# swook/EVE

Measured on AMD Instinct MI355X. Metric: train-step frames/sec, 128x128 eye patches T=30, higher is better.
Workload: dtype bf16; 1 GPU; BASELINE configs[1]: EyeNet training (configs/eye_net.json: ResNet-18-IN + GRU-128, angular + pupil L1 losses, clip 5.0, Adam wd 0.005), 128x128 patches, fwd+bwd+clip+Adam; global_batch=32, batch_per_gpu=32, seq_len=30, parallelism=dp1

## Files before the change

eve_amd/csrc/conv_igemm.hip:

```cpp
#include <limits.h>
#include <stdio.h>
#include <stdlib.h>

#include <initializer_list>
#include <type_traits>
#include "common.h"

namespace eve {

struct GatherParams {
    int N, IH, IW, Cin;
    int OH, OW, Cout;
    int KH, KW;
    int o_mul, k_mul, off, div;
    int K;
    uint32_t M;
    FastDiv fd_ohw, fd_ow, fd_cin, fd_kw, fd_oh;
};

template <typename T>
__device__ __forceinline__ uint4 prologue_vec(uint4 q, const float* __restrict__ ssp, int act) {
    constexpr int VEC = Elem<T>::VEC;
    float f[VEC];
    Elem<T>::unpack(q, f);
    const float4* s4 = reinterpret_cast<const float4*>(ssp);
#pragma unroll
    for (int e = 0; e < VEC / 2; ++e) {
        float4 s = s4[e];
        f[2 * e] = act_fwd(f[2 * e] * s.x + s.y, act);
        f[2 * e + 1] = act_fwd(f[2 * e + 1] * s.z + s.w, act);
    }
    return Elem<T>::pack(f);
}

template <typename T> struct Mma {
    __device__ static __forceinline__ void run(f32x4_t& acc, const uint4& a, const uint4& b) { Elem<T>::mfma(acc, a, b); }
};
template <> struct Mma<float> {
    __device__ static __forceinline__ void run(f32x4_t& acc, const uint4& a, const uint4& b) {
        acc = __builtin_amdgcn_mfma_f32_16x16x4f32(__builtin_bit_cast(float, a.x), __builtin_bit_cast(float, b.x), acc, 0, 0, 0);
        acc = __builtin_amdgcn_mfma_f32_16x16x4f32(__builtin_bit_cast(float, a.y), __builtin_bit_cast(float, b.y), acc, 0, 0, 0);
        acc = __builtin_amdgcn_mfma_f32_16x16x4f32(__builtin_bit_cast(float, a.z), __builtin_bit_cast(float, b.z), acc, 0, 0, 0);
        acc = __builtin_amdgcn_mfma_f32_16x16x4f32(__builtin_bit_cast(float, a.w), __builtin_bit_cast(float, b.w), acc, 0, 0, 0);
    }
};

}
#include "conv_fast.h"
#include "conv_wg8.h"
#include "conv_wg8s2.h"
#include "conv_ws64.h"
#include "conv_1x1.h"
#include "conv_3x3s.h"
#include "wgrad_halo.h"
#include "wgrad_wg8.h"
namespace eve {

template <typename T, int NT, bool PRO>
__global__ __launch_bounds__(256) void igemm_kernel(const GatherParams p, const T* __restrict__ src,
                                                    const T* __restrict__ w,
                                                    const float* __restrict__ bias,
                                                    const float* __restrict__ ss, const int pro_act,
                                                    const int epi_act, T* __restrict__ out) {
    constexpr int VEC = Elem<T>::VEC;
    constexpr int BM = 128, BN = 32 * NT, BK = 8 * VEC;
    __shared__ uint4 lds[2 * (BM + BN) * 8];

    const int tid = threadIdx.x;
    const uint32_t tiles_n = (p.Cout + BN - 1) / BN;
    const uint32_t lid = xcd_remap(blockIdx.x, gridDim.x);
    const uint32_t m0 = (lid / tiles_n) * BM;
    const uint32_t n0 = (lid % tiles_n) * BN;

    const int v = tid & 7;
    const int r0 = tid >> 3;
    int a_y0[4], a_x0[4], a_pix[4], a_n[4];
    bool a_ok[4];
#pragma unroll
    for (int j = 0; j < 4; ++j) {
        const uint32_t m = m0 + r0 + 32 * j;
        a_ok[j] = m < p.M;
        const uint32_t mm = a_ok[j] ? m : 0;
        const uint32_t n = fd_div(mm, p.fd_ohw);
        const uint32_t rem = mm - n * (uint32_t)(p.OH * p.OW);
        const uint32_t oy = fd_div(rem, p.fd_ow);
        const uint32_t ox = rem - oy * (uint32_t)p.OW;
        a_y0[j] = (int)oy * p.o_mul + p.off;
        a_x0[j] = (int)ox * p.o_mul + p.off;
        a_pix[j] = (int)n * p.IH * p.IW;
        a_n[j] = (int)n;
    }

    uint4 ra[4], rb[NT];

    auto load_tile = [&](int kt) {
        const uint32_t kvec = (uint32_t)kt * BK + (uint32_t)v * VEC;
        const bool kvalid = kvec < (uint32_t)p.K;
        const uint32_t tap = fd_div(kvec, p.fd_cin);
        const int ci = (int)(kvec - tap * (uint32_t)p.Cin);
        const uint32_t kh = fd_div(tap, p.fd_kw);
        const int kw = (int)(tap - kh * (uint32_t)p.KW);
        const int dy = (int)kh * p.k_mul, dx = kw * p.k_mul;
#pragma unroll
        for (int j = 0; j < 4; ++j) {
            int sy = a_y0[j] + dy, sx = a_x0[j] + dx;
            bool ok = a_ok[j] && kvalid && sy >= 0 && sx >= 0;
            if (p.div > 1) {
                ok = ok && (sy % p.div == 0) && (sx % p.div == 0);
                sy /= p.div;
                sx /= p.div;
            }
            ok = ok && sy < p.IH && sx < p.IW;
            uint4 q = make_uint4(0, 0, 0, 0);
            if (ok) {
                const size_t e = ((size_t)(a_pix[j] + sy * p.IW + sx)) * (size_t)p.Cin + (size_t)ci;
                q = *reinterpret_cast<const uint4*>(src + e);
                if (PRO) q = prologue_vec<T>(q, ss + ((size_t)a_n[j] * p.Cin + ci) * 2, pro_act);
            }
            ra[j] = q;
        }
#pragma unroll
        for (int j = 0; j < NT; ++j) {
            const uint32_t co = n0 + r0 + 32 * j;
            uint4 q = make_uint4(0, 0, 0, 0);
            if (kvalid && co < (uint32_t)p.Cout)
                q = *reinterpret_cast<const uint4*>(w + (size_t)co * p.K + kvec);
            rb[j] = q;
        }
    };
    auto store_tile = [&](int buf) {
        uint4* base = lds + buf * (BM + BN) * 8;
#pragma unroll
        for (int j = 0; j < 4; ++j) {
            const int row = r0 + 32 * j;
            base[row * 8 + (v ^ (row & 7))] = ra[j];
        }
#pragma unroll
        for (int j = 0; j < NT; ++j) {
            const int row = r0 + 32 * j;
            base[BM * 8 + row * 8 + (v ^ (row & 7))] = rb[j];
        }
    };

    const int lane = tid & 63, wv = tid >> 6;
    const int wm = wv >> 1, wn = wv & 1;
    const int li = lane & 15, lg = lane >> 4;

    f32x4_t acc[4][NT];
#pragma unroll
    for (int a = 0; a < 4; ++a)
#pragma unroll
        for (int b = 0; b < NT; ++b) acc[a][b] = f32x4_t{0.f, 0.f, 0.f, 0.f};

    constexpr bool SPLIT_SUM = std::is_same<T, float>::value;
    constexpr int FLUSH = 8;
    f32x4_t tot[SPLIT_SUM ? 4 : 1][SPLIT_SUM ? NT : 1];
    if (SPLIT_SUM) {
#pragma unroll
        for (int a = 0; a < 4; ++a)
#pragma unroll
            for (int b = 0; b < NT; ++b) tot[SPLIT_SUM ? a : 0][SPLIT_SUM ? b : 0] = f32x4_t{0.f, 0.f, 0.f, 0.f};
    }

    const int nk = (p.K + BK - 1) / BK;
    load_tile(0);
    store_tile(0);
    __syncthreads();
    for (int kt = 0; kt < nk; ++kt) {
        const int cur = kt & 1;
        const bool more = kt + 1 < nk;
        if (more) load_tile(kt + 1);
        if (SPLIT_SUM && kt > 0 && (kt % FLUSH) == 0) {
#pragma unroll
            for (int a = 0; a < 4; ++a)
#pragma unroll
                for (int b = 0; b < NT; ++b) {
                    tot[SPLIT_SUM ? a : 0][SPLIT_SUM ? b : 0] += acc[a][b];
                    acc[a][b] = f32x4_t{0.f, 0.f, 0.f, 0.f};
                }
        }
        const uint4* la = lds + cur * (BM + BN) * 8;
        const uint4* lb = la + BM * 8;
#pragma unroll
        for (int c = 0; c < 2; ++c) {
            const int vc = c * 4 + lg;
            uint4 fx[4], fw[NT];
#pragma unroll
            for (int mt = 0; mt < 4; ++mt) {
                const int row = wm * 64 + mt * 16 + li;
                fx[mt] = la[row * 8 + (vc ^ (row & 7))];
            }
#pragma unroll
            for (int nt = 0; nt < NT; ++nt) {
                const int row = wn * 16 * NT + nt * 16 + li;
                fw[nt] = lb[row * 8 + (vc ^ (row & 7))];
            }
#pragma unroll
            for (int mt = 0; mt < 4; ++mt)
#pragma unroll
                for (int nt = 0; nt < NT; ++nt) Mma<T>::run(acc[mt][nt], fw[nt], fx[mt]);
        }
        if (more) store_tile(cur ^ 1);
        __syncthreads();
    }

    if (SPLIT_SUM) {
#pragma unroll
        for (int a = 0; a < 4; ++a)
// ... 410 lines not shown
        tp.ntaps = p.KH * p.KW;
        for (int kh = 0; kh < p.KH; ++kh)
            for (int kw = 0; kw < p.KW; ++kw) {
                const int t = kh * p.KW + kw;
                tp.dy[t] = (signed char)(kh * p.k_mul); tp.dx[t] = (signed char)(kw * p.k_mul); tp.wt[t] = (signed char)t;
            }
        tp.osy = tp.osx = 1; tp.oy0 = tp.ox0 = 0; tp.OHf = p.OH; tp.OWf = p.OW;
        launch_dma_one<T>(p, tp, src, w, bias, epi_act, out, (uint32_t)src_bytes, (uint32_t)w_bytes, s);
        return true;
    }
    if (p.o_mul != 1 || p.k_mul != -1 || bias || (epi_act & 0xff) != EVE_ACT_NONE) return false;
    const int sd = p.div;
    bool need_zero = false;
    for (int pass = 0; pass < 2; ++pass) {
        for (int py = 0; py < sd; ++py)
            for (int px = 0; px < sd; ++px) {
                TapPlan tp;
                tp.ntaps = 0;
                for (int kh = 0; kh < p.KH; ++kh)
                    for (int kw = 0; kw < p.KW; ++kw) {
                        const int ny = py + p.off - kh, nx = px + p.off - kw;
                        if (ny % sd != 0 || nx % sd != 0) continue;
                        tp.dy[tp.ntaps] = (signed char)(ny / sd); tp.dx[tp.ntaps] = (signed char)(nx / sd);
                        tp.wt[tp.ntaps] = (signed char)(kh * p.KW + kw);
                        ++tp.ntaps;
                    }
                const int sub_h = (p.OH - py + sd - 1) / sd, sub_w = (p.OW - px + sd - 1) / sd;
                if (sub_h <= 0 || sub_w <= 0) continue;
                if (tp.ntaps == 0) { need_zero = true; continue; }
                if (pass == 0) continue;
                GatherParams q = p;
                q.OH = sub_h; q.OW = sub_w;
                q.o_mul = 1; q.off = 0; q.div = 1;
                q.M = (uint32_t)((long long)p.N * sub_h * sub_w);
                q.fd_ohw = make_fastdiv(sub_h * sub_w); q.fd_ow = make_fastdiv(sub_w);
                tp.osy = tp.osx = sd; tp.oy0 = py; tp.ox0 = px; tp.OHf = p.OH; tp.OWf = p.OW;
                launch_dma_one<T>(q, tp, src, w, bias, epi_act, out, (uint32_t)src_bytes, (uint32_t)w_bytes, s);
            }
        if (pass == 0 && need_zero && !(epi_act & EVE_EPI_ACC))
            (void)hipMemsetAsync(out, 0, (size_t)p.N * p.OH * p.OW * p.Cout * sizeof(T), s);
    }
    return true;
}

template <typename T>
static int launch_igemm(const GatherParams& p, const void* src, const void* w, const float* bias,
                        const float* ss, int pro_act, int epi_act, void* out, hipStream_t s) {
    if (!ss && !use_v1() && launch_igemm_dma<T>(p, src, w, bias, epi_act, out, s)) return 0;
    const bool wide = p.Cout > 64;
    const uint32_t bn = wide ? 128 : 64;
    const uint32_t tiles = ((p.M + 127) / 128) * ((p.Cout + bn - 1) / bn);
    dim3 grid(tiles), block(256);
    const T* a = (const T*)src; const T* b = (const T*)w; T* o = (T*)out;
    if (wide) {
        if (ss) EVE_LAUNCH("igemm_kernel<T, 4, true>", (igemm_kernel<T, 4, true>), grid, block, 0, s, p, a, b, bias, ss, pro_act, epi_act, o);
        else    EVE_LAUNCH("igemm_kernel<T, 4, false>", (igemm_kernel<T, 4, false>), grid, block, 0, s, p, a, b, bias, ss, pro_act, epi_act, o);
    } else {
        if (ss) EVE_LAUNCH("igemm_kernel<T, 2, true>", (igemm_kernel<T, 2, true>), grid, block, 0, s, p, a, b, bias, ss, pro_act, epi_act, o);
        else    EVE_LAUNCH("igemm_kernel<T, 2, false>", (igemm_kernel<T, 2, false>), grid, block, 0, s, p, a, b, bias, ss, pro_act, epi_act, o);
    }
    return 0;
}

static void wgrad_split(const GatherParams& p, uint32_t tk, uint32_t tc, size_t lds_per_wg, uint32_t& splits, uint32_t& rows) {
    const int target_env = g_cfg.wgrad_target_wgs;
    uint32_t per_cu = lds_per_wg ? (uint32_t)((160 * 1024) / lds_per_wg) : 3;
    per_cu = per_cu < 1 ? 1 : (per_cu > 3 ? 3 : per_cu);
    const uint32_t target = target_env > 0 ? (uint32_t)target_env : 256u * per_cu;
    uint32_t want = target / (tk * tc);
    const int min_rows = g_cfg.wgrad_min_rows;
    uint32_t max_splits = (p.M + (uint32_t)min_rows - 1) / (uint32_t)min_rows;
    splits = want < 1 ? 1 : (want > max_splits ? max_splits : want);
    if (splits < 1) splits = 1;
    if (splits > 65535) splits = 65535;
    rows = (p.M + splits - 1) / splits;
    rows = (rows + 63) / 64 * 64;
    splits = (p.M + rows - 1) / rows;
}

template <typename HT>
static bool launch_wgrad_halo(const GatherParams& p, const void* x, const void* dy, float* dw, float* db, hipStream_t s) {
    if (!g_cfg.wgrad_halo) return false;
    const int ks = p.KH;
    if ((ks != 3 && ks != 1) || p.KW != ks || p.o_mul != 1 || p.k_mul != 1 || p.off != -(ks / 2) || p.div != 1 || p.OH != p.IH ||
        p.OW != p.IW)
        return false;
    const int W = p.IW, H = p.IH;
    const long long min_m = g_cfg.wgrad_halo_min_m;
    if (W < 32 || W > 128 || (W & (W - 1)) || p.Cin % 16 || p.Cout % 16 || (long long)p.M < min_m) return false;
    const int MT = p.Cout / 16, CT = p.Cin / 16;
    const bool split = ks == 3 && MT == 4 && CT == 4;
    if (ks == 3 && !split && !((MT == 1 && (CT == 1 || CT == 2 || CT == 4)) || (MT == 2 && (CT == 1 || CT == 2)))) return false;
    if (ks == 1 && !((MT == 2 && CT == 1) || (MT == 1 && CT == 4) || (MT == 1 && CT == 2) || (MT == 4 && CT == 2) || (MT == 2 && CT == 4)))
        return false;
    const unsigned long long xb = (unsigned long long)p.N * H * W * p.Cin * 2, db_ = (unsigned long long)p.M * p.Cout * 2;
    if (xb >= (1ull << 31) || db_ >= (1ull << 31)) return false;
    const size_t red = (size_t)(ks * ks * p.Cin * p.Cout + p.Cout) * 4;
    const unsigned occ = (ks == 3 && MT * CT >= 4) ? 2 : 3;
    int TH = 0; size_t lds = 0;
    int nreg = 0;
    if (split) {
        const int force_th = g_cfg.wg64_th, force_nreg = g_cfg.wg64_nreg;
        for (int th : {8, 4, 2, 1}) {
            if (force_th && th != force_th) continue;
            const size_t need = (size_t)(th + 2) * (W + 2) * 128 + (size_t)th * W * 128;
            for (int nr : {3, 2}) {
                if (force_nreg && nr != force_nreg) continue;
                if (nr * need <= (size_t)160 * 1024) { TH = th; nreg = nr; lds = nr * need > red ? nr * need : red; break; }
            }
            if (TH) break;
        }
    } else
    for (size_t budget : {(size_t)(occ == 3 ? 52 : 78) * 1024, (size_t)78 * 1024}) {
        for (int th : {4, 2, 1}) {
            const size_t need = (size_t)(th + ks - 1) * (W + ks - 1) * p.Cin * 2 + (size_t)th * W * p.Cout * 2;
            if (need <= budget && need >= red) { TH = th; lds = need; break; }
        }
        if (TH) break;
    }
    if (!TH) return false;
    WgradHaloParams h;
    h.N = p.N; h.H = H; h.W = W; h.TH = TH; h.bands = (H + TH - 1) / TH;
    h.total_bands = (uint32_t)p.N * h.bands; h.x_bytes = (uint32_t)xb; h.dy_bytes = (uint32_t)db_;
    h.log2_cpr = 0; h.nreg = nreg;
    while ((32 << h.log2_cpr) < W) ++h.log2_cpr;
    const unsigned per_cu = (unsigned)((160 * 1024) / lds);
    unsigned grid = 256 * (per_cu > occ ? occ : per_cu);
    if (grid > h.total_bands) grid = h.total_bands;
    auto band_tile = [&](auto kernel) { launch(kernel, dim3(grid), dim3(256), lds, s, h, (const HT*)x, (const HT*)dy, dw, db); };
    if (split) {
        const unsigned g64 = h.total_bands < 256u ? h.total_bands : 256u;
        const int fixed64 = g_cfg.wg64_fixed;
        if (fixed64 && W == 32 && TH == 8 && H % 8 == 0)
            EVE_LAUNCH(EVE_HNAME(HT, "wgrad_halo64_kernel<", ", fixed>"), (wgrad_halo64_kernel<HT, true>), dim3(g64), dim3(512), lds, s, h, (const HT*)x, (const HT*)dy, dw, db);
        else
            EVE_LAUNCH(EVE_HNAME(HT, "wgrad_halo64_kernel<", ">"), (wgrad_halo64_kernel<HT, false>), dim3(g64), dim3(512), lds, s, h, (const HT*)x, (const HT*)dy, dw, db);
    } else if (ks == 3) {
        if (MT == 1 && CT == 1) band_tile(EVE_KERNEL_H(HT, wgrad_halo_kernel, 1, 1, 3));
        else if (MT == 1 && CT == 2) band_tile(EVE_KERNEL_H(HT, wgrad_halo_kernel, 1, 2, 3));
        else if (MT == 1 && CT == 4) band_tile(EVE_KERNEL_H(HT, wgrad_halo_kernel, 1, 4, 3));
        else if (MT == 2 && CT == 1) band_tile(EVE_KERNEL_H(HT, wgrad_halo_kernel, 2, 1, 3));
        else band_tile(EVE_KERNEL_H(HT, wgrad_halo_kernel, 2, 2, 3));
    } else {
        if (MT == 2 && CT == 1) band_tile(EVE_KERNEL_H(HT, wgrad_halo_kernel, 2, 1, 1));
        else if (MT == 1 && CT == 4) band_tile(EVE_KERNEL_H(HT, wgrad_halo_kernel, 1, 4, 1));
        else if (MT == 1 && CT == 2) band_tile(EVE_KERNEL_H(HT, wgrad_halo_kernel, 1, 2, 1));
        else if (MT == 4 && CT == 2) band_tile(EVE_KERNEL_H(HT, wgrad_halo_kernel, 4, 2, 1));
        else band_tile(EVE_KERNEL_H(HT, wgrad_halo_kernel, 2, 4, 1));
    }
    return true;
}

#define EVE_WGRAD_TR(T, WCO, WK, P2, MT) EVE_HNAME(T, "wgrad_tr_kernel<", ", " #WCO ", " #WK ", " #P2 ", mt" #MT ">"), ic<WCO>{}, ic<WK>{}, ic<P2>{}, ic<MT>{}

template <typename T>
static int launch_wgrad(const GatherParams& p, const void* x, const void* dy, const float* ss, int pro_act,
                        float* dw, hipStream_t s, float* db = nullptr, void* workspace = nullptr, unsigned long long workspace_bytes = 0) {
    if constexpr (sizeof(T) == 2) {
    if (!ss && !use_v1() && launch_wgrad_halo<T>(p, x, dy, dw, db, s)) return db ? 1 : 0;
    if (!ss && !use_v1()) {
        const unsigned long long x_bytes = (unsigned long long)p.N * p.IH * p.IW * p.Cin * 2;
        const unsigned long long dy_bytes = (unsigned long long)p.M * p.Cout * 2;
        if (x_bytes < (1ull << 31) && dy_bytes < (1ull << 31)) {
            uint32_t splits, rows;
            const bool pow2 = ((p.OW & (p.OW - 1)) == 0) && ((p.OH & (p.OH - 1)) == 0);
            auto lds_bytes = [](int bco, int bkk, int mode) { return (size_t)((bco == 128 || (bkk == 256 && mode == 2)) ? 3 : 4) * 32 * (bco + bkk) * 2; };
            auto tr_tile = [&](const char* name, auto wco, auto wk, auto p2, auto mt, uint32_t tk, uint32_t tc) {
                constexpr int WCO = decltype(wco)::value, WK = decltype(wk)::value, P2 = decltype(p2)::value, MT = decltype(mt)::value;
                auto go = [&](auto kernel) {
                    launch(kernel, dim3(tk * tc * splits), dim3(64 * WCO * WK), lds_bytes(64 * WCO, 64 * WK, P2), s, p, (const T*)x, (const T*)dy, dw,
                           rows, (uint32_t)x_bytes, (uint32_t)dy_bytes, db);
                };
                if (db) go(Named<wgrad_tr_kernel<T, WCO, WK, P2, true, MT>>{name});
                else    go(Named<wgrad_tr_kernel<T, WCO, WK, P2, false, MT>>{name});
            };
            const bool pow2w = (p.OW & (p.OW - 1)) == 0;
            const int mode = pow2 ? 1 : ((pow2w && p.OH * p.OW >= 32) ? 2 : 0);
            const int wg8w = g_cfg.wgrad_wg8;
            if (wg8w && !db && mode == 1 && p.Cout % 256 == 0 && p.K % 256 == 0) {
                const uint32_t tk = p.K / 256, tc = p.Cout / 256;
                wgrad_split(p, tk, tc, (size_t)128 * 1024, splits, rows);
                const unsigned long long n = (unsigned long long)p.Cout * p.K;
                const bool slab = splits > 1 && workspace && (unsigned long long)splits * n * 4 <= workspace_bytes && ((uintptr_t)dw & 15) == 0 &&
                                  ((uintptr_t)workspace & 15) == 0;
                if (slab) {
                    EVE_LAUNCH(EVE_HNAME(T, "wgrad_wg8_kernel<", ", true>"), (wgrad_wg8_kernel<T, true>), dim3(tk * tc * splits), dim3(512), (size_t)128 * 1024, s, p,
                               (const T*)x, (const T*)dy, (float*)workspace, rows, (uint32_t)x_bytes, (uint32_t)dy_bytes);
                    const long long n4 = (long long)(n / 4);
                    long long blocks = (n4 + 255) / 256;
                    if (blocks > 2048) blocks = 2048;
                    hipLaunchKernelGGL(wgrad_slab_reduce_kernel, dim3((unsigned)blocks), dim3(256), 0, s, (const float*)workspace, dw, n4, (int)splits);
                } else {
                    EVE_LAUNCH(EVE_HNAME(T, "wgrad_wg8_kernel<", ", false>"), (wgrad_wg8_kernel<T, false>), dim3(tk * tc * splits), dim3(512), (size_t)128 * 1024, s, p,
                               (const T*)x, (const T*)dy, dw, rows, (uint32_t)x_bytes, (uint32_t)dy_bytes);
                }
            } else if (p.Cout > 64) {
                const uint32_t tk = (p.K + 127) / 128, tc = (p.Cout + 127) / 128;
                wgrad_split(p, tk, tc, lds_bytes(128, 128, mode), splits, rows);
                if (mode == 1)      tr_tile(EVE_WGRAD_TR(T, 2, 2, 1, 4), tk, tc);
                else if (mode == 2) tr_tile(EVE_WGRAD_TR(T, 2, 2, 2, 4), tk, tc);
                else                tr_tile(EVE_WGRAD_TR(T, 2, 2, 0, 4), tk, tc);
            } else if (mode == 1 && p.K % 192 == 0 && p.K <= 1152) {
                const uint32_t tk = p.K / 192;
                wgrad_split(p, tk, 1, lds_bytes(64, 192, mode), splits, rows);
                tr_tile(EVE_WGRAD_TR(T, 1, 3, 1, 4), tk, 1);
            } else {
                const uint32_t tk = (p.K + 255) / 256, tc = 1;
                wgrad_split(p, tk, tc, lds_bytes(64, 256, mode), splits, rows);
                if (mode == 1)      tr_tile(EVE_WGRAD_TR(T, 1, 4, 1, 4), tk, tc);
                else if (mode == 2) {
                    if (p.Cout <= 16)      tr_tile(EVE_WGRAD_TR(T, 1, 4, 2, 1), tk, tc);
                    else if (p.Cout <= 32) tr_tile(EVE_WGRAD_TR(T, 1, 4, 2, 2), tk, tc);
                    else                   tr_tile(EVE_WGRAD_TR(T, 1, 4, 2, 4), tk, tc);
                }
                else                tr_tile(EVE_WGRAD_TR(T, 1, 4, 0, 4), tk, tc);
            }
            return db ? 1 : 0;
        }
    }
    }
    const bool wide = p.Cout > 64;
    const uint32_t bco = wide ? 128 : 64;
    const uint32_t tk = (p.K + 127) / 128, tc = (p.Cout + bco - 1) / bco;
    uint32_t want = (1024 + tk * tc - 1) / (tk * tc);
    uint32_t max_splits = (p.M + 255) / 256;
    uint32_t splits = want < 1 ? 1 : (want > max_splits ? max_splits : want);
    if (splits < 1) splits = 1;
    if (splits > 65535) splits = 65535;
    uint32_t rows = (p.M + splits - 1) / splits;
    rows = (rows + 63) / 64 * 64;
    splits = (p.M + rows - 1) / rows;
    dim3 grid(tk, tc, splits), block(256);
    const T* a = (const T*)x; const T* b = (const T*)dy;
    if (wide) {
        if (ss) EVE_LAUNCH("wgrad_kernel<T, 4, true>", (wgrad_kernel<T, 4, true>), grid, block, 0, s, p, a, b, ss, pro_act, dw, rows);
        else    EVE_LAUNCH("wgrad_kernel<T, 4, false>", (wgrad_kernel<T, 4, false>), grid, block, 0, s, p, a, b, ss, pro_act, dw, rows);
    } else {
        if (ss) EVE_LAUNCH("wgrad_kernel<T, 2, true>", (wgrad_kernel<T, 2, true>), grid, block, 0, s, p, a, b, ss, pro_act, dw, rows);
        else    EVE_LAUNCH("wgrad_kernel<T, 2, false>", (wgrad_kernel<T, 2, false>), grid, block, 0, s, p, a, b, ss, pro_act, dw, rows);
    }
    return 0;
}

template <typename HT>
static bool launch_s2_fwd_wg8(const eve_conv_desc* d, const void* x, const void* w, const float* bias, int epi_act, void* y, hipStream_t s) {
    const int on = g_cfg.conv_wg8, min_tiles = g_cfg.conv_wg8_s2_min_tiles;
    const int W = d->OW;
    if (!on || d->KH != 3 || d->KW != 3 || d->stride != 2 || d->pad != 1 || d->OH != W || d->IH != 2 * W || d->IW != 2 * W ||
        !(W == 16 || W == 8 || W == 4) || d->Cin % 64 || (epi_act & ~0xff) ||
        !((epi_act & 0xff) == EVE_ACT_NONE || (epi_act & 0xff) == EVE_ACT_RELU))
        return false;
    const int cout_t = W == 16 ? 128 : 256;
    if (d->Cout % cout_t) return false;
    const unsigned long long xb = (unsigned long long)d->N * 4 * W * W * d->Cin * 2, wb = (unsigned long long)d->Cout * 9 * d->Cin * 2;
    if (xb >= (1ull << 31) || wb >= (1ull << 31)) return false;
    const int ti = W == 16 ? 2 : (W == 8 ? 4 : 16);
    const uint32_t tiles = (uint32_t)((d->N + ti - 1) / ti) * (uint32_t)(d->Cout / cout_t);
    if ((int)tiles < min_tiles) return false;
    Wg8Params g;
    g.N = d->N; g.Cin = d->Cin; g.Cout = d->Cout; g.flip = 0; g.K = 9 * d->Cin; g.x_bytes = (uint32_t)xb; g.w_bytes = (uint32_t)wb;
    g.tiles_n = (uint32_t)(d->Cout / cout_t); g.s2_py = 0;
    auto s2_tile = [&](auto kernel, auto geom) {
        launch(kernel, dim3(tiles), dim3(512), decltype(geom)::LDS, s, g, (const HT*)x, (const HT*)w, bias, epi_act, (HT*)y);
    };
    if (W == 16) s2_tile(EVE_KERNEL_H(HT, conv3x3s2_wg8_kernel, 4, 2, 16), Wg8S2Geom<4, 2, 16>{});
    else if (W == 8) s2_tile(EVE_KERNEL_H(HT, conv3x3s2_wg8_kernel, 2, 4, 8), Wg8S2Geom<2, 4, 8>{});
    else s2_tile(EVE_KERNEL_H(HT, conv3x3s2_wg8_kernel, 2, 4, 4), Wg8S2Geom<2, 4, 4>{});
    return true;
}

template <typename H>
__global__ __launch_bounds__(256) void s2_dgrad_pack_kernel(const H* __restrict__ w_ihwo, H* __restrict__ w0, H* __restrict__ w1,
                                                            int Cdx, int Cout) {
    const int kv = Cout / 8;
    const long long n0 = (long long)2 * Cdx * 2 * kv, n1 = (long long)2 * Cdx * 4 * kv;
    for (long long i = (long long)blockIdx.x * 256 + threadIdx.x; i < n0 + n1; i += (long long)gridDim.x * 256) {
        const int py = i >= n0 ? 1 : 0, nt = py ? 4 : 2;
        const long long r = py ? i - n0 : i;
        const int v = (int)(r % kv), t = (int)((r / kv) % nt), row = (int)(r / ((long long)kv * nt));
        const int px = row >= Cdx ? 1 : 0, ci = row - px * Cdx;
        const int dy = py ? t >> 1 : 0, dx = t & 1;
        const int kh = py + 1 - 2 * dy, kw = px + 1 - 2 * dx;
        uint4 q = make_uint4(0u, 0u, 0u, 0u);
        if (kh >= 0 && kw >= 0)
            q = reinterpret_cast<const uint4*>(w_ihwo + (((size_t)ci * 3 + kh) * 3 + kw) * Cout)[v];
        reinterpret_cast<uint4*>(py ? w1 : w0)[r] = q;
    }
}

#define EVE_S2_DGRAD(H, WM, WN, W, NT) eve::Named<conv3x3_wg8_kernel<H, WM, WN, W, NT>>{EVE_HNAME(H, "conv3x3_wg8_kernel<", ", " #WM ", " #WN ", " #W ", s2dgrad" #NT ">")}, Wg8Geom<WM, WN, W>{}, ic<NT>{}

template <typename HT>
static bool launch_s2_dgrad_wg8(const eve_conv_desc* d, const void* dy, const void* w_ihwo, void* dx, void* workspace,
                                unsigned long long workspace_bytes, hipStream_t s) {
    const int on = g_cfg.conv_wg8, min_tiles = g_cfg.conv_wg8_s2_min_tiles;
    const int W = d->OW, Cdx = d->Cin, Co = d->Cout;
    if (!on || d->KH != 3 || d->KW != 3 || d->stride != 2 || d->pad != 1 || d->OH != W || d->IH != 2 * W || d->IW != 2 * W ||
        !(W == 16 || W == 8 || W == 4) || Co % 64 || !workspace || ((uintptr_t)workspace & 255))
        return false;
    const int cout_t = W == 16 ? 128 : 256;
    if ((2 * Cdx) % cout_t) return false;
    const unsigned long long wbytes = (unsigned long long)2 * Cdx * 6 * Co * 2;
    const unsigned long long xb = (unsigned long long)d->N * W * W * Co * 2, ob = (unsigned long long)d->N * 4 * W * W * Cdx * 2;
    if (wbytes > workspace_bytes || xb >= (1ull << 31) || ob >= (1ull << 31) || wbytes >= (1ull << 31)) return false;
    const int ti = W == 16 ? 2 : (W == 8 ? 4 : 16);
    const uint32_t tiles = (uint32_t)((d->N + ti - 1) / ti) * (uint32_t)(2 * Cdx / cout_t);
    if ((int)tiles < min_tiles) return false;
    HT* w0 = (HT*)workspace;
    HT* w1 = w0 + (size_t)2 * Cdx * 2 * Co;
    const long long nvec = (long long)2 * Cdx * 6 * (Co / 8);
    hipLaunchKernelGGL(s2_dgrad_pack_kernel<HT>, dim3((unsigned)((nvec + 255) / 256 > 1024 ? 1024 : (nvec + 255) / 256)), dim3(256), 0, s,
                       (const HT*)w_ihwo, w0, w1, Cdx, Co);
    Wg8Params g;
    g.N = d->N; g.Cin = Co; g.Cout = 2 * Cdx; g.flip = 0; g.x_bytes = (uint32_t)xb; g.tiles_n = (uint32_t)(2 * Cdx / cout_t);
    auto row_parity = [&](auto kernel, auto geom, auto nt, const HT* wp, int py) {
        constexpr int NT = decltype(nt)::value;
        g.K = NT * Co; g.w_bytes = (uint32_t)((unsigned long long)2 * Cdx * NT * Co * 2); g.s2_py = py;
        launch(kernel, dim3(tiles), dim3(512), decltype(geom)::LDS, s, g, (const HT*)dy, wp, (const float*)nullptr, (int)EVE_ACT_NONE, (HT*)dx);
    };
    if (W == 16) { row_parity(EVE_S2_DGRAD(HT, 4, 2, 16, 2), w0, 0); row_parity(EVE_S2_DGRAD(HT, 4, 2, 16, 4), w1, 1); }
    else if (W == 8) { row_parity(EVE_S2_DGRAD(HT, 2, 4, 8, 2), w0, 0); row_parity(EVE_S2_DGRAD(HT, 2, 4, 8, 4), w1, 1); }
    else { row_parity(EVE_S2_DGRAD(HT, 2, 4, 4, 2), w0, 0); row_parity(EVE_S2_DGRAD(HT, 2, 4, 4, 4), w1, 1); }
    return true;
}

static int conv_entry(const char* who, const eve_conv_desc* d, const char* cout_msg, bool operands, int max_cout_vecs = INT_MAX) {
    const int vec = (d && d->dtype != EVE_DT_F32) ? 8 : 4;
    if (int e = check_desc(d, vec)) return e;
    char msg[128];
    if (cout_msg && (d->Cout % vec || d->Cout / vec > max_cout_vecs)) { snprintf(msg, sizeof(msg), "%s: %s", who, cout_msg); return set_error_msg(msg); }
    if (!operands) { snprintf(msg, sizeof(msg), "%s: null pointer", who); return set_error_msg(msg); }
    return 0;
}

struct ConvCall {
    const char* who;
    const eve_conv_desc* d;
    bool dgrad;
    const void* in; const void* w; const float* bias; int epi_act; void* out;
    const float* in_scale_shift; int pro_act;
    void* workspace; unsigned long long workspace_bytes;
    hipStream_t s;
    int cin() const { return dgrad ? d->Cout : d->Cin; }
    int cout() const { return dgrad ? d->Cin : d->Cout; }
};
typedef bool (*ConvRung)(const ConvCall&);

static bool rung_1x1_stream(const ConvCall& c) {
// ... 155 lines not shown
```

Before: 89070 frames/s.

## Add 128x384-tile wgrad kernel for 3x3 Cin=128 convs with wide slab reduce

Adds a specialised weight-gradient kernel for 3x3 convolutions with 128 input channels. It uses a 128(Cout) x 384(K) tile with a 4-slot LDS DMA pipeline and split lead/follow wave scheduling. Split-K partial results go either to per-split slabs, summed by a new wide reduce kernel that parallelises over splits, or directly through atomics. It is gated on the wgrad_wg8 config knob and on a minimum M, and its intent is better MFMA reuse for the layer3-sized convs. The cost is another specialised path with its own correctness surface.

```diff
diff --git a/eve_amd/csrc/conv_igemm.hip b/eve_amd/csrc/conv_igemm.hip
--- a/eve_amd/csrc/conv_igemm.hip
+++ b/eve_amd/csrc/conv_igemm.hip
@@ -54,6 +54,7 @@
 #include "conv_3x3s.h"
 #include "wgrad_halo.h"
 #include "wgrad_wg8.h"
+#include "wgrad_wg8_t128.h"
 namespace eve {
 
 template <typename T, int NT, bool PRO>
@@ -770,6 +771,8 @@
 }
 
 #define EVE_WGRAD_TR(T, WCO, WK, P2, MT) EVE_HNAME(T, "wgrad_tr_kernel<", ", " #WCO ", " #WK ", " #P2 ", mt" #MT ">"), ic<WCO>{}, ic<WK>{}, ic<P2>{}, ic<MT>{}
+
+static constexpr uint32_t WGRAD_WG8_T128_MIN_M = 65536;
 
 template <typename T>
 static int launch_wgrad(const GatherParams& p, const void* x, const void* dy, const float* ss, int pro_act,
@@ -812,6 +815,23 @@
                     EVE_LAUNCH(EVE_HNAME(T, "wgrad_wg8_kernel<", ", false>"), (wgrad_wg8_kernel<T, false>), dim3(tk * tc * splits), dim3(512), (size_t)128 * 1024, s, p,
                                (const T*)x, (const T*)dy, dw, rows, (uint32_t)x_bytes, (uint32_t)dy_bytes);
                 }
+            } else if ((wg8w == 1 || wg8w == 2) && !db && mode == 1 && p.KH == 3 && p.KW == 3 && p.Cin == 128 && p.Cout % 128 == 0 &&
+                       (wg8w == 2 || p.M >= WGRAD_WG8_T128_MIN_M)) {
+                const uint32_t tk = 3, tc = p.Cout / 128;
+                wgrad_split(p, tk, tc, (size_t)128 * 1024, splits, rows);
+                const unsigned long long n = (unsigned long long)p.Cout * p.K;
+                const bool slab = splits > 1 && workspace && (unsigned long long)splits * n * 4 <= workspace_bytes && ((uintptr_t)dw & 15) == 0 &&
+                                  ((uintptr_t)workspace & 15) == 0;
+                if (slab) {
+                    EVE_LAUNCH(EVE_HNAME(T, "wgrad_wg8_t128_kernel<", ", true>"), (wgrad_wg8_t128_kernel<T, true>), dim3(tk * tc * splits), dim3(512), (size_t)128 * 1024,
+                               s, p, (const T*)x, (const T*)dy, (float*)workspace, rows, (uint32_t)x_bytes, (uint32_t)dy_bytes);
+                    const long long n4 = (long long)(n / 4);
+                    hipLaunchKernelGGL(wgrad_slab_reduce_wide_kernel, dim3((unsigned)((n4 + 31) / 32)), dim3(256), 0, s, (const float*)workspace, dw, n4,
+                                       (int)splits);
+                } else {
+                    EVE_LAUNCH(EVE_HNAME(T, "wgrad_wg8_t128_kernel<", ", false>"), (wgrad_wg8_t128_kernel<T, false>), dim3(tk * tc * splits), dim3(512), (size_t)128 * 1024,
+                               s, p, (const T*)x, (const T*)dy, dw, rows, (uint32_t)x_bytes, (uint32_t)dy_bytes);
+                }
             } else if (p.Cout > 64) {
                 const uint32_t tk = (p.K + 127) / 128, tc = (p.Cout + 127) / 128;
                 wgrad_split(p, tk, tc, lds_bytes(128, 128, mode), splits, rows);
diff --git a/eve_amd/csrc/wgrad_wg8_t128.h b/eve_amd/csrc/wgrad_wg8_t128.h
--- /dev/null
+++ b/eve_amd/csrc/wgrad_wg8_t128.h
@@ -0,0 +1,206 @@
+#pragma once
+#include "common.h"
+#include "lds_dma.h"
+#include "conv_fast.h"
+
+namespace eve {
+
+template <typename H, bool SLAB>
+__global__ __launch_bounds__(512, 2) void wgrad_wg8_t128_kernel(const GatherParams p, const H* __restrict__ x,
+                                                                const H* __restrict__ dy, float* __restrict__ dw,
+                                                                const uint32_t rows_per_split, const uint32_t x_bytes,
+                                                                const uint32_t dy_bytes) {
+    constexpr int WK = 4;
+    constexpr int BCO = 128, BKK = 384;
+    constexpr int PROW = BCO * 2, QROW = BKK * 2;
+    constexpr int PSL = PROW / 16, QSL = QROW / 16;
+    constexpr int STEP = 32, NT = 512;
+    constexpr int QJ = STEP * QSL / NT;
+    constexpr int QBASE = STEP * PROW;
+    constexpr int BUF = STEP * (PROW + QROW);
+    static_assert(STEP * PSL == NT && STEP * QSL == QJ * NT && BUF == 32768, "slot count per thread");
+    extern __shared__ __attribute__((aligned(16))) char lds[];
+
+    const int tid = threadIdx.x;
+    const int wave = __builtin_amdgcn_readfirstlane(tid >> 6);
+    const uint32_t tk = (uint32_t)p.K / BKK, tc = (uint32_t)p.Cout / BCO;
+    const uint32_t lid = tk * tc >= 4 ? xcd_remap(blockIdx.x, gridDim.x) : blockIdx.x;
+    const uint32_t k0 = (lid % tk) * BKK, co0 = ((lid / tk) % tc) * BCO;
+    const uint32_t m_begin = (lid / (tk * tc)) * rows_per_split;
+    const uint32_t m_end = min(p.M, m_begin + rows_per_split);
+
+    const eve_int4 rs_x = make_rsrc_words(x, x_bytes);
+    const eve_int4 rs_dy = make_rsrc_words(dy, dy_bytes);
+    const uint32_t lds0 = lds_addr_of(lds);
+
+    const int cin2 = p.Cin * 2, cout2 = p.Cout * 2;
+    const int sh_w = __builtin_ctz((unsigned)p.OW), sh_hw = __builtin_ctz((unsigned)(p.OH * p.OW));
+    int p_row, p_const, q_row[QJ], q_const[QJ], q_ty[QJ], q_tx[QJ];
+    {
+        const int row = tid / PSL, sl = tid % PSL;
+        const int sg = sl ^ (tr_key<PROW>(row) << 1);
+        p_row = row;
+        p_const = row * cout2 + (int)(co0 + sg * 8) * 2;
+    }
+#pragma unroll
+    for (int j = 0; j < QJ; ++j) {
+        const int q = tid + NT * j;
+        const int row = q / QSL, sl = q % QSL;
+        const int sg = sl ^ (tr_key<QROW>(row) << 1);
+        q_row[j] = row;
+        const uint32_t k = k0 + sg * 8;
+        const uint32_t tap = fd_div(k, p.fd_cin), kh = fd_div(tap, p.fd_kw);
+        const int col = (int)(k - tap * (uint32_t)p.Cin) * 2;
+        const int ddy = (int)kh * p.k_mul + p.off, ddx = (int)(tap - kh * (uint32_t)p.KW) * p.k_mul + p.off;
+        const uint32_t r = (uint32_t)row;
+        const int n_t = (int)(r >> sh_hw), oy_t = (int)((r >> sh_w) & (uint32_t)(p.OH - 1)), ox_t = (int)(r & (uint32_t)(p.OW - 1));
+        q_ty[j] = oy_t * p.o_mul + ddy;
+        q_tx[j] = ox_t * p.o_mul + ddx;
+        q_const[j] = ((n_t * p.IH + q_ty[j]) * p.IW + q_tx[j]) * cin2 + col;
+    }
+    auto offsets = [&](uint32_t mbase, int& vp, int* vq) {
+        const uint32_t left = m_end > mbase ? m_end - mbase : 0u;
+        const int pbase = (int)mbase * cout2;
+        const uint32_t n_s = mbase >> sh_hw, oy_s = (mbase >> sh_w) & (uint32_t)(p.OH - 1), ox_s = mbase & (uint32_t)(p.OW - 1);
+        const int sy0 = (int)oy_s * p.o_mul, sx0 = (int)ox_s * p.o_mul;
+        const int qbase = (((int)n_s * p.IH + sy0) * p.IW + sx0) * cin2;
+        vp = (uint32_t)p_row < left ? pbase + p_const : EVE_OOB;
+#pragma unroll
+        for (int j = 0; j < QJ; ++j) {
+            const bool ok = ((uint32_t)q_row[j] < left) & ((uint32_t)(sy0 + q_ty[j]) < (uint32_t)p.IH) &
+                            ((uint32_t)(sx0 + q_tx[j]) < (uint32_t)p.IW);
+            vq[j] = ok ? qbase + q_const[j] : EVE_OOB;
+        }
+    };
+    auto issue = [&](int slot, const int vp, const int* vq) {
+        const uint32_t pb = lds0 + slot * BUF, qb = pb + QBASE;
+        lds_dma16_asm(rs_dy, pb + wave * 64 * 16, vp);
+#pragma unroll
+        for (int j = 0; j < QJ; ++j) lds_dma16_asm(rs_x, qb + (wave * 64 + NT * j) * 16, vq[j]);
+    };
+
+    const int lane = tid & 63;
+    const int wco = wave / WK, wk = wave % WK;
+    const int t = lane & 15, g = lane >> 4;
+    const int lrow = 8 * g + (t >> 2);
+    const int key = tr_key<PROW>(lrow);
+    static_assert(PROW % 256 == 0 && QROW % 256 == 0, "one key for both operands");
+    const int half = (t & 1) * 8, hs = (t & 3) >> 1;
+    uint32_t poff[4], qoff[6];
+#pragma unroll
+    for (int i = 0; i < 4; ++i) poff[i] = lds0 + lrow * PROW + (((wco * 8 + i * 2 + hs) ^ (key << 1)) * 16) + half;
+#pragma unroll
+    for (int i = 0; i < 6; ++i) qoff[i] = lds0 + QBASE + lrow * QROW + (((wk * 12 + i * 2 + hs) ^ (key << 1)) * 16) + half;
+
+    f32x4_t acc[6][4];
+#pragma unroll
+    for (int b = 0; b < 6; ++b)
+#pragma unroll
+        for (int c = 0; c < 4; ++c) acc[b][c] = f32x4_t{0.f, 0.f, 0.f, 0.f};
+
+    if (m_begin < m_end) {
+        const int nsteps = (int)((m_end - m_begin + STEP - 1) / STEP);
+        const bool lead = wave < 4;
+        int vp, vq[QJ];
+        offsets(m_begin, vp, vq);
+        issue(0, vp, vq);
+        offsets(m_begin + STEP, vp, vq);
+        issue(1, vp, vq);
+        asm volatile("s_waitcnt vmcnt(0)" ::: "memory");
+        __builtin_amdgcn_s_barrier();
+        if (!lead) __builtin_amdgcn_s_setprio(2);
+        uint4 fp[4], fq[6];
+#pragma unroll
+        for (int i = 0; i < 4; ++i) fp[i] = make_uint4(0u, 0u, 0u, 0u);
+#pragma unroll
+        for (int i = 0; i < 6; ++i) fq[i] = make_uint4(0u, 0u, 0u, 0u);
+        auto mma = [&]() {
+#pragma unroll
+            for (int i = 0; i < 6; ++i) mma4_inplace_b<H>(acc[i], fp, fq[i]);
+        };
+        auto step = [&](int st, auto slot_c) {
+            constexpr int SLOT = decltype(slot_c)::value;
+            if (!lead) mma();
+            constexpr int SB = SLOT * BUF;
+            constexpr int HI = SB >= 65536 ? 65536 : 0;
+            static_assert(SB - HI + 4 * QROW < 65536 && SB - HI + 4 * PROW < 65536, "immediate range");
+#pragma unroll
+            for (int i = 0; i < 4; ++i) {
+                const uint2 a0 = lds_tr_read<SB - HI>(poff[i] + HI);
+                const uint2 a1 = lds_tr_read<SB - HI + 4 * PROW>(poff[i] + HI);
+                fp[i] = make_uint4(a0.x, a0.y, a1.x, a1.y);
+            }
+#pragma unroll
+            for (int i = 0; i < 6; ++i) {
+                const uint2 b0 = lds_tr_read<SB - HI>(qoff[i] + HI);
+                const uint2 b1 = lds_tr_read<SB - HI + 4 * QROW>(qoff[i] + HI);
+                fq[i] = make_uint4(b0.x, b0.y, b1.x, b1.y);
+            }
+            offsets(m_begin + (uint32_t)(st + 2) * STEP, vp, vq);
+            issue((SLOT + 2) & 3, vp, vq);
+            if (lead) mma();
+            asm volatile("s_waitcnt vmcnt(4)" ::: "memory");
+            __builtin_amdgcn_s_barrier();
+        };
+        int st = 0;
+        for (; st + 4 <= nsteps; st += 4) {
+            step(st, std::integral_constant<int, 0>{});
+            step(st + 1, std::integral_constant<int, 1>{});
+            step(st + 2, std::integral_constant<int, 2>{});
+            step(st + 3, std::integral_constant<int, 3>{});
+        }
+        if (st < nsteps) step(st, std::integral_constant<int, 0>{});
+        if (st + 1 < nsteps) step(st + 1, std::integral_constant<int, 1>{});
+        if (st + 2 < nsteps) step(st + 2, std::integral_constant<int, 2>{});
+        if (!lead) mma();
+        __builtin_amdgcn_s_setprio(0);
+        asm volatile("s_waitcnt vmcnt(0)" ::: "memory");
+    }
+    asm volatile("s_nop 15\n\ts_nop 15"
+                 : "+a"(acc[0][0]), "+a"(acc[0][1]), "+a"(acc[0][2]), "+a"(acc[0][3]), "+a"(acc[1][0]), "+a"(acc[1][1]),
+                   "+a"(acc[1][2]), "+a"(acc[1][3]), "+a"(acc[2][0]), "+a"(acc[2][1]), "+a"(acc[2][2]), "+a"(acc[2][3]) :: "memory");
+    asm volatile("s_nop 15\n\ts_nop 15"
+                 : "+a"(acc[3][0]), "+a"(acc[3][1]), "+a"(acc[3][2]), "+a"(acc[3][3]), "+a"(acc[4][0]), "+a"(acc[4][1]),
+                   "+a"(acc[4][2]), "+a"(acc[4][3]), "+a"(acc[5][0]), "+a"(acc[5][1]), "+a"(acc[5][2]), "+a"(acc[5][3]) :: "memory");
+    float* const dst = SLAB ? dw + (size_t)(lid / (tk * tc)) * ((size_t)p.Cout * p.K) : dw;
+#pragma unroll
+    for (int kt = 0; kt < 6; ++kt) {
+        const uint32_t k = k0 + wk * 96 + kt * 16 + t;
+#pragma unroll
+        for (int mt = 0; mt < 4; ++mt)
+#pragma unroll
+            for (int r = 0; r < 4; ++r) {
+                const uint32_t co = co0 + wco * 64 + mt * 16 + g * 4 + r;
+                if (SLAB) dst[(size_t)co * p.K + k] = acc[kt][mt][r];
+                else atomicAdd(dst + (size_t)co * p.K + k, acc[kt][mt][r]);
+            }
+    }
+}
+
+__global__ __launch_bounds__(256) void wgrad_slab_reduce_wide_kernel(const float* __restrict__ slabs, float* __restrict__ dw,
+                                                                     const long long n4, const int splits) {
+    __shared__ float4 part[8][32];
+    const int c = threadIdx.x & 31, q = threadIdx.x >> 5;
+    const long long i = (long long)blockIdx.x * 32 + c;
+    float4 a = make_float4(0.f, 0.f, 0.f, 0.f);
+    if (i < n4) {
+#pragma unroll 4
+        for (int s = q; s < splits; s += 8) {
+            const float4 b = reinterpret_cast<const float4*>(slabs)[(long long)s * n4 + i];
+            a.x += b.x; a.y += b.y; a.z += b.z; a.w += b.w;
+        }
+    }
+    part[q][c] = a;
+    __syncthreads();
+    if (q == 0 && i < n4) {
+        float4 r = reinterpret_cast<const float4*>(dw)[i];
+#pragma unroll
+        for (int j = 0; j < 8; ++j) {
+            const float4 b = part[j][c];
+            r.x += b.x; r.y += b.y; r.z += b.z; r.w += b.w;
+        }
+        reinterpret_cast<float4*>(dw)[i] = r;
+    }
+}
+
+}
```

Measured after the change: 90200 frames/s (median of 6 runs). 1.01x the previous value.
